# guomc9/CudaRayTracing

Measured on AMD Instinct MI355X. Metric: Mrays/sec, higher is better.
Workload: dtype f32

## Files before the change

cudaraytracing_amd/_capi.py:

```python
import ctypes as C
import os

import numpy as np

from . import build as _build

CRT_OK = 0
ERR_INVALID_ARG, ERR_NO_DEVICE, ERR_HIP = -1, -2, -3
TRAVERSAL_EXACT = 0
TRAVERSAL_REFERENCE = 1
TRAVERSAL_FAST = 2
FLAG_STATS = 1
FLAG_TILED_OUTPUT = 2
FLAG_FORCE_EXACT = 4
FLAG_TRACE_ALL = 8
FLAG_BOUNDED_RADIANCE = 16
FLAG_VARIANCE = 32
GATHER_AUTO, GATHER_RCCL, GATHER_COPY = 0, 1, 2
INTERSECT_RAW_DIRECTIONS, INTERSECT_FORCE_EXACT, INTERSECT_VISIBILITY = 0x100, 0x200, 0x400
TILE = 8


class CrtError(RuntimeError):
    def __init__(self, status, where, detail):
# ... 130 lines not shown
                ("width", C.c_uint32), ("height", C.c_uint32), ("bvh_thresh_n", C.c_uint32),
                ("light_sample_n", C.c_uint32), ("spp", C.c_uint32), ("p_rr", C.c_float)]


NODE_DTYPE = np.dtype([("lc", "<i4"), ("rc", "<i4"), ("n", "<u4"), ("it", "<i4"), ("aa", "<f4", 3), ("bb", "<f4", 3)])
TRI_DTYPE = np.dtype([("v1", "<f4", 3), ("v2", "<f4", 3), ("v3", "<f4", 3), ("normal", "<f4", 3), ("area", "<f4"),
                      ("area_of_obj", "<f4"), ("material", "<i4")])
MAT_DTYPE = np.dtype([("kd", "<f4", 3), ("ke", "<f4", 3), ("ns", "<f4"), ("mode", "<i4"), ("has_emit", "<i4")])
LIGHT_DTYPE = np.dtype([("first_tri", "<u4"), ("count", "<u4")])

ABI_VERSION = 5

EXPORTS = ["crt_strerror", "crt_last_error", "crt_abi_version", "crt_device_count", "crt_scene_create",
           "crt_scene_accel_info", "crt_scene_destroy", "crt_task_obj", "crt_shard_slots", "crt_render", "crt_render_device", "crt_render_range", "crt_render_range_device", "crt_last_launch_ms", "crt_radiance_storage", "crt_preview", "crt_preview_device", "crt_variance", "crt_variance_device", "crt_render_aov", "crt_render_aov_device", "crt_denoise_defaults", "crt_denoise_scratch_bytes", "crt_denoise", "crt_denoise_device", "crt_denoise_var_defaults", "crt_denoise_var", "crt_denoise_var_device", "crt_multi_create", "crt_multi_destroy",
           "crt_multi_render", "crt_multi_frame_device", "crt_intersect",
           "crt_device_math", "crt_device_philox", "crt_device_rcp_check", "crt_scene_export", "crt_host_scene_create", "crt_host_scene_destroy",
           "crt_host_scene_add_obj", "crt_host_scene_set_bvh", "crt_host_scene_set_bvh_device", "crt_host_scene_desc", "crt_host_scene_num_objects",
           "crt_host_scene_object", "crt_inverse_view", "crt_task_load", "crt_image_load", "crt_write_png", "crt_write_pfm"]

_lib = None


def lib_path():
    return _build.LIB


def lib():
    global _lib
    if _lib is not None:
        return _lib
    path = os.environ.get("CRT_LIB_PATH") or _build.build_lib()
# ... 33 lines not shown
    L.crt_denoise_var_defaults.argtypes = [C.POINTER(DenoiseParams)]
    L.crt_denoise_var.argtypes = [C.c_int, C.POINTER(DenoiseParams), C.POINTER(DenoiseVarInputs), C.c_void_p, C.c_void_p, C.c_void_p,
                                  C.POINTER(DenoiseInfo)]
    L.crt_denoise_var_device.argtypes = [C.c_int, C.POINTER(DenoiseParams), C.POINTER(DenoiseVarInputs), C.c_void_p, C.c_void_p, C.c_void_p,
                                         C.c_void_p, C.c_uint64, C.c_void_p, C.POINTER(DenoiseInfo)]
    L.crt_multi_create.argtypes = [C.POINTER(SceneDesc), C.POINTER(C.c_int), C.c_uint32, C.c_uint32, C.POINTER(C.c_void_p)]
    L.crt_multi_destroy.argtypes = [C.c_void_p]
    L.crt_multi_render.argtypes = [C.c_void_p, C.POINTER(Camera), C.POINTER(Params), C.c_void_p, C.c_void_p, C.POINTER(Stats),
                                   C.POINTER(MultiInfo)]
    L.crt_multi_frame_device.argtypes = [C.c_void_p, C.POINTER(C.c_void_p), C.POINTER(C.c_void_p), C.POINTER(C.c_int)]
    L.crt_intersect.argtypes = [C.c_void_p, C.c_uint32, C.c_void_p, C.c_void_p, C.c_uint32, C.c_void_p, C.c_void_p]
    L.crt_device_math.argtypes = [C.c_int, C.c_char_p, C.c_uint32, C.c_void_p, C.c_void_p, C.c_void_p]
    L.crt_device_philox.argtypes = [C.c_int, C.c_uint32, C.c_void_p, C.c_void_p, C.c_void_p]
    L.crt_device_rcp_check.argtypes = [C.c_int, C.POINTER(C.c_uint64), C.POINTER(C.c_uint64)]
    L.crt_scene_export.argtypes = [C.c_void_p, C.c_char_p, C.c_void_p, C.c_size_t, C.POINTER(C.c_size_t)]
    L.crt_host_scene_create.argtypes = [C.c_uint32, C.c_uint32, C.POINTER(C.c_void_p)]
    L.crt_host_scene_destroy.argtypes = [C.c_void_p]
    L.crt_host_scene_add_obj.argtypes = [C.c_void_p, C.c_char_p, C.c_char_p]
    L.crt_host_scene_set_bvh.argtypes = [C.c_void_p, C.c_uint32]
    L.crt_host_scene_set_bvh_device.argtypes = [C.c_void_p, C.c_uint32, C.c_int, C.POINTER(BvhBuildInfo)]
    L.crt_host_scene_desc.argtypes = [C.c_void_p, C.POINTER(SceneDesc)]
    L.crt_host_scene_num_objects.argtypes = [C.c_void_p, C.POINTER(C.c_uint32)]
    L.crt_host_scene_object.argtypes = [C.c_void_p, C.c_uint32, C.POINTER(C.c_float), C.POINTER(C.c_int32),
                                        C.POINTER(C.c_uint32)]
    L.crt_inverse_view.argtypes = [C.c_void_p, C.c_void_p, C.c_void_p, C.c_void_p]
    L.crt_task_load.argtypes = [C.c_char_p, C.POINTER(Task)]
    L.crt_task_obj.argtypes = [C.c_char_p, C.c_uint32, C.c_char_p, C.c_char_p, C.c_uint32]
    L.crt_image_load.argtypes = [C.c_char_p, C.POINTER(C.c_int32), C.POINTER(C.c_int32), C.POINTER(C.c_int32), C.c_void_p, C.c_uint64]
    L.crt_write_png.argtypes = [C.c_char_p, C.c_uint32, C.c_uint32, C.c_void_p]
    L.crt_write_pfm.argtypes = [C.c_char_p, C.c_uint32, C.c_uint32, C.c_uint32, C.c_void_p]
# ... 19 lines not shown
```

cudaraytracing_amd/api.py:

```python
import ctypes as C
import math
import os

import numpy as np

from . import _capi as capi


def get_inverse_view_matrix(eye_pos, lookat, up):
    e = np.asarray(eye_pos, dtype=np.float32)
    l = np.asarray(lookat, dtype=np.float32)
    u = np.asarray(up, dtype=np.float32)
    out = np.zeros(9, dtype=np.float32)
    capi.check(capi.lib().crt_inverse_view(capi.ptr(e), capi.ptr(l), capi.ptr(u), capi.ptr(out)), "crt_inverse_view")
    return out


def fov_to_radians(fov_y_deg):
    return np.float32(np.float32(np.float32(fov_y_deg) * np.float32(math.pi)) / np.float32(180))


class Task:

    def __init__(self, config_path, base_dir=None):
# ... 60 lines not shown
        buf = (C.c_char * (n * dtype.itemsize)).from_address(C.addressof(p.contents))
        return np.frombuffer(buf, dtype=dtype).copy()

    def nodes(self):
        d = self.desc()
        return self._arr(d.nodes, d.n_nodes, capi.NODE_DTYPE)

    def triangles(self):
        d = self.desc()
        return self._arr(d.tris, d.n_tris, capi.TRI_DTYPE)

    def light_triangles(self):
        d = self.desc()
        return self._arr(d.light_tris, d.n_light_tris, capi.TRI_DTYPE)

    def materials(self):
        d = self.desc()
        return self._arr(d.materials, d.n_materials, capi.MAT_DTYPE)

    def lights(self):
        d = self.desc()
        return self._arr(d.lights, d.n_lights, capi.LIGHT_DTYPE)

    @property
    def root(self):
        return int(self.desc().root)

    def objects(self):
        n = C.c_uint32()
        capi.check(capi.lib().crt_host_scene_num_objects(self._h, C.byref(n)), "crt_host_scene_num_objects")
# ... 44 lines not shown
        self.denoise_info = None
        self.variance_buffer = None

    def _handle(self, what):
        if not self._h:
            raise RuntimeError("%s: no single-device scene handle (freed, or a MultiRender)" % what)
        return self._h

    def accel_info(self):
        self._handle("accel_info")
        a = capi.AccelInfo()
        capi.check(capi.lib().crt_scene_accel_info(self._h, C.byref(a)), "crt_scene_accel_info")
        return a.as_dict()

    EXPORT_ARRAYS = {"nodes": np.float32, "nodes3": np.float32, "nodes4": np.float32, "nodes4i": np.float32, "leaf_geo": np.float32,
                     "leaf_geo_i": np.float32, "rec_map": np.int32, "tri_geo": np.float32, "leaf_count": np.int32, "tri_nm": np.float32}

    def export_trees(self):
        h = self._handle("export_trees")
        L = capi.lib()
        out = {}
        for name, dt in self.EXPORT_ARRAYS.items():
            n = C.c_size_t()
            capi.check(L.crt_scene_export(h, name.encode(), None, 0, C.byref(n)), "crt_scene_export")
            a = np.zeros(n.value // np.dtype(dt).itemsize, dtype=dt)
            if n.value:
                capi.check(L.crt_scene_export(h, name.encode(), capi.ptr(a), a.nbytes, C.byref(n)), "crt_scene_export")
            out[name] = a.reshape(-1, 4) if dt is np.float32 else a
        s = capi.TreeScalars()
        n = C.c_size_t()
        capi.check(L.crt_scene_export(h, b"scalars", C.byref(s), C.sizeof(s), C.byref(n)), "crt_scene_export")
# ... 446 lines not shown
```

cudaraytracing_amd/csrc/crt_device.h:

```cpp
#ifndef CRT_DEVICE_H
#define CRT_DEVICE_H

#include <hip/hip_runtime.h>
#include <stdint.h>

#include "crt_detmath.h"

namespace crtdev {

#define CRT_EPSILON 0.00001f
#define CRT_BOUNCE_STACK_SIZE 64
#define CRT_TILE 8

#define NODE4I_F4 6
#define TNM_MAT(w_) ((w_) & 0x3fffffffu)
#define TNM_EMITTER(w_) (((w_) >> 30) & 1u)
#define TNM_SPECULAR(w_) ((w_) >> 31)

struct DevScene {
    const float4* nodes;
    const float4* tri_geo;
    const int32_t* tri_mat;
    const float4* mats;
    const float4* ltri;
    const uint4* lights;
    const int32_t* leaf_count;
    int32_t root_fast;
    int32_t root_exact;
    int32_t n_lights;
    const float4* nodes3;
    const float4* leaf_geo;
    int32_t root3_fast, root3_exact;
// ... 92 lines not shown
```

cudaraytracing_amd/csrc/crt_mega3.hip:

```cpp
#include "crt_internal.h"

#include <cstdio>
#include <cstdlib>
#include <cstring>
#include <vector>

namespace crtk {

struct NewRay {
    F3 o, d;
    float tl;
    uint32_t kind, flags;
};

__device__ __forceinline__ float fmin3(float a, float b, float c) { return __builtin_fminf(__builtin_fminf(a, b), c); }
__device__ __forceinline__ float fmax3(float a, float b, float c) { return __builtin_fmaxf(__builtin_fmaxf(a, b), c); }
__device__ __forceinline__ v2f v2(float a, float b) { v2f r; r.x = a; r.y = b; return r; }
__device__ __forceinline__ v2f v2s(float a) { v2f r; r.x = a; r.y = a; return r; }

__device__ __forceinline__ int smax(const int a, const int b)
{
    int r;
    asm("s_max_i32 %0, %1, %2" : "=s"(r) : "s"(a), "s"(b) : "scc");
    return r;
// ... 128 lines not shown
            if (v - j >= 0) {
                F3 ind = mul3(L, f3(fm[j].x, fm[j].y, fm[j].z));
                ind = scale3(ind, cs[j]);
                ind = scale3(ind, inv_pdf_sphere);
                ind = div3(ind, P.p_rr);
                L = add3(ind, f3(a[j].x, a[j].y, a[j].z));
            }
        }
    }
    return L;
}

__device__ __forceinline__ bool shadow_blocked_bit(const bool tl_inf, const int tri) { return tri >= 0 || tl_inf; }
#define ST_TL_INF (1u << 12)

template <int MODE, bool RING = false>
__device__ __forceinline__ uint32_t logic_A(const LParams& P, const Tables<false>& tb, const uint32_t g, const float4 qa, const float4 qb, NewRay& nr,
                                            PathCounters& cnt, const bool trace_all)
{
    const DevScene& sc = P.sc;
    const Pool& pl = P.pool;
    constexpr bool TRI_CC = MODE != 1;
    const float4 la = gld(&pl.la[g]);
    const uint4 idv = load_path_id<RING, !TRI_CC>(P, g);
    const float4 cc = gld(&pl.cc[g]);
    const uint32_t st = __float_as_uint(la.w);
    const uint32_t stage = (st >> 8) & 15u;
    const uint32_t vtri_old = TRI_CC ? ((st & 0xfffu) == ((uint32_t)ST_HIT << 8) ? 0u : __float_as_uint(cc.w)) : idv.w;
    const float4 vn = gld(&sc.tri_nm[vtri_old]);
    const float res_t = qa.w;
    const int res_tri = __float_as_int(qb.w);
    const float4 gq_hit = gld(&sc.tri_nm[res_tri >= 0 ? res_tri : 0]);
    const uint32_t mat_old = min(TNM_MAT(__float_as_uint(vn.w)), P.n_mats - 1u);
    const uint32_t mat_cur = stage == ST_HIT ? TNM_MAT(__float_as_uint(gq_hit.w)) : mat_old;
    uint32_t tnm_cur = stage == ST_HIT ? __float_as_uint(gq_hit.w) : __float_as_uint(vn.w);
    float4 m0_cur = mat_row(tb, mat_cur, 0);
    const uint32_t n_nee = (uint32_t)(sc.n_lights * P.lsn);
    const uint32_t q_next = stage == ST_SHADOW ? (st >> 16) + 1 : 0u;
    uint4 lg_next = make_uint4(0u, 1u, 0u, 0u);
    if (n_nee > 0) {
        if (sc.n_lights == 1) {
            const crt_u4v_ l0_ = *(const __attribute__((address_space(4))) crt_u4v_*)tb.lights;
            lg_next = make_uint4(l0_.x, l0_.y, l0_.z, l0_.w);
        } else lg_next = gld(&tb.lights[fast_div(q_next < n_nee ? q_next : 0u, P.lsn_div.m, P.lsn_div.sh)]);
    }
    Lane s;
    s.depth = st & 255u; s.q = st >> 16; s.stage = stage;
    s.Ld = f3(la.x, la.y, la.z);
    s.nrm = f3(vn.x, vn.y, vn.z); s.mat = TNM_MAT(__float_as_uint(vn.w));
    s.pixel_index = idv.x; s.k = idv.y; s.item = idv.z;
    s.ro = f3(qa.x, qa.y, qa.z); s.tl = 0.0f;
    s.rd = f3(qb.x, qb.y, qb.z);
    s.pos = s.ro; s.vtri = vtri_old; s.c = f3(0.0f, 0.0f, 0.0f); s.kind = RAY_NONE;
    bool do_enter = false;
    if (stage == ST_SHADOW) {
        const bool blocked = TRI_CC ? shadow_blocked_bit((st & ST_TL_INF) != 0u, res_tri) : shadow_blocked<MODE>(cc.w, res_t, res_tri);
        if (!blocked) s.Ld = add3(s.Ld, f3(cc.x, cc.y, cc.z));
        s.q++;
    } else if (stage == ST_HIT) {
// ... 62 lines not shown
        if (TNM_SPECULAR(tnm_cur)) gst_rec(&pl.rec_b[(size_t)s.depth * pl.n + g], make_float4(s.rd.x, s.rd.y, s.rd.z, 0.0f));
        if (!TRI_CC) store_path_tri(P, g, s.vtri);
        if (TNM_EMITTER(tnm_cur)) {
            gst(&pl.la[g], make_float4(TRI_CC ? __uint_as_float(s.vtri) : 0.0f, 0.0f, 0.0f, __uint_as_float(s.depth | ((uint32_t)ST_FIN << 8) | (1u << 16))));
            return PH3_LC;
        }
        s.Ld = f3(0.0f, 0.0f, 0.0f);
        s.q = 0;
        if (n_nee == 0) {
            gst(&pl.la[g], make_float4(0.0f, 0.0f, 0.0f, __uint_as_float(s.depth | ((uint32_t)ST_NEED << 8))));
            if (TRI_CC) gst(&pl.cc[g].w, __uint_as_float(s.vtri));
            nr.o = s.pos;
            return PH3_LB;
        }
    }
    constexpr int LA_LOOP_MIN = 16;
    const float4 m0 = m0_cur;
    bool skip;
    for (bool first = true;; first = false) {
        if (first) setup_shadow_lg(P, s, f3(m0.x, m0.y, m0.z), lg_next);
        else setup_shadow(P, tb, s, f3(m0.x, m0.y, m0.z));
        skip = MODE != 1 && !trace_all && (s.c.x == 0.0f && s.c.y == 0.0f && s.c.z == 0.0f);
        if (!skip) break;
        cnt.untraced++;
        if (__popcll(__builtin_amdgcn_ballot_w64(true)) < LA_LOOP_MIN) break;
        cnt.rays++; cnt.shadow++;
        s.q++;
        if (s.q == n_nee) {
            gst(&pl.la[g], make_float4(s.Ld.x, s.Ld.y, s.Ld.z, __uint_as_float(s.depth | ((uint32_t)ST_NEED << 8))));
            if (TRI_CC) gst(&pl.cc[g].w, __uint_as_float(s.vtri));
            nr.o = s.pos;
            return PH3_LB;
        }
    }
    gst(&pl.la[g], make_float4(s.Ld.x, s.Ld.y, s.Ld.z, __uint_as_float(s.depth | ((uint32_t)ST_SHADOW << 8) | (s.q << 16) | ((TRI_CC && s.tl == pinf()) ? ST_TL_INF : 0u))));
    gst(&pl.cc[g], make_float4(s.c.x, s.c.y, s.c.z, TRI_CC ? __uint_as_float(s.vtri) : s.tl));
    nr.o = s.ro; nr.d = s.rd; nr.tl = s.tl; nr.kind = RAY_SHADOW;
    nr.flags = RF_SHADOW | (s.q + 1 == n_nee ? RF_LAST : 0u) | (skip ? RF_SKIP : 0u);
    return PH3_NONE;
}

template <int MODE, bool RING = false>
__device__ __forceinline__ uint32_t logic_B(const LParams& P, const uint32_t g, const float4 qa, const float4 qb, NewRay& nr)
{
    const Pool& pl = P.pool;
    constexpr bool TRI_CC = MODE != 1;
    const float4 la = gld(&pl.la[g]);
    const uint4 idv = load_path_id<RING, !TRI_CC>(P, g);
// ... 949 lines not shown
        } else {
            leaf_arm(std::true_type{});
        }
        }
      }
        if (act == PH3_NONE && !(commit_ring && (__builtin_amdgcn_readfirstlane((int)S.waitq) & 0xff) != 0)) break;
        STAMP_OTHER()
        if (act == PH3_LA) {
            POP3(PH3_LA)
            bool new_exact = false;
            if (on) {
                LOGIC_PARAMS()
                NewRay nr;
                float4 ra_, rb_;
                ray_result(S, id, ra_, rb_);
                nph = logic_A<MODE, RING>(Pl, tl, g, ra_, rb_, nr, cnt, ALL);
                if (nph == PH3_LB) { S.A[id].x = nr.o.x; S.A[id].y = nr.o.y; S.A[id].z = nr.o.z; }
                if (nph == PH3_NONE) nph = start_ray<MODE, false, LDS3, IMPL>(Pl.sc, S, id, nr, cnt, M3.force_exact != 0, new_exact);
            }
            n_exact += (int)__popcll(__ballot(new_exact));
            PUSH3()
            STAMP(0)
        } else if (act == PH3_LB) {
            POP3(PH3_LB)
            bool new_exact = false;
            if (on) {
                LOGIC_PARAMS()
                NewRay nr;
                float4 ra_, rb_;
                ray_result(S, id, ra_, rb_);
                nph = logic_B<MODE, RING>(Pl, g, ra_, rb_, nr);
// ... 94 lines not shown
            atomicAdd(&cs[C_TESTS], (unsigned long long)c);
            atomicAdd(&cs[C_HITS], (unsigned long long)d);
            atomicMax(&cs[C_MAXSP], (unsigned long long)ms);
            for (int p = 0; p < 5; p++) {
                atomicAdd(&cs[C_DIAG + 2 * p], (unsigned long long)dg_b[p]);
                atomicAdd(&cs[C_DIAG + 2 * p + 1], (unsigned long long)dg_l[p]);
            }
        }
        for (int k = 0; k < 6; k++) {
            const uint32_t v = wave_sum(dg_sp[k]);
            if (lane == 0) atomicAdd(&cs[C_DIAG + 10 + k], (unsigned long long)v);
        }
        for (int k = 0; k < 2; k++) {
            const uint32_t v = wave_sum(dg_ov[k]);
            if (lane == 0) atomicAdd(&cs[C_DIAG + 16 + k], (unsigned long long)v);
        }
    }
}

template <bool RING>
__global__ __launch_bounds__(64) void k_order_items(const LParams P, uint32_t* list, unsigned int* cnt)
{
    const uint32_t spans = (P.order_window + 1023u) / 1024u;
    const uint32_t sh = blockIdx.x / spans, sp = blockIdx.x - sh * spans;
    const uint32_t slo = sh * P.items_per_shard;
    if (slo >= P.n_items) return;
    const uint32_t hi = min(slo + P.items_per_shard, P.n_items);
    const uint32_t lo = hi - min(P.order_window, hi - slo);
    const uint32_t b = lo + sp * 1024u;
    if (b >= hi) return;
// ... 132 lines not shown
```

cudaraytracing_amd/csrc/crt_path.h:

```cpp
#ifndef CRT_PATH_H
#define CRT_PATH_H
#include "../../include/crt.h"
#include "crt_accel.h"
#include "crt_device.h"
#include "crt_trace.h"

#include <hip/hip_runtime.h>

#include <cfloat>
#include <cstddef>
#include <cstdint>
#include <type_traits>

namespace crtk {
using namespace crtdev;

enum { C_RAYS = 0, C_SHADOW, C_PROBE, C_INNER, C_LEAF, C_TESTS, C_HITS, C_PATHS, C_ALIVE, C_MAXSP, C_SUMSP, C_CYC_LOGIC, C_CYC_LEAF, C_CYC_INNER, C_CYC_OTHER,
       C_DIAG , C_UNTRACED = C_DIAG + 20, C_COUNT };
#define CNT_SHARDS 256
#define CNT_STRIDE 40
#define ITEM_SHARDS 64
#define ITEM_STRIDE 32

enum { ST_DEAD = 0, ST_NEW = 1, ST_HIT = 2, ST_PROBE = 3, ST_SHADOW = 4, ST_FIN = 5, ST_NEED = 6, ST_WAIT = 7, ST_COUNT_ };
// ... 134 lines not shown
        const int src = __ffsll((long long)found) - 1;
        const uint32_t sh = (uint32_t)__builtin_amdgcn_readlane((int)look, src);
        const int leader = __ffsll((long long)mask) - 1;
        unsigned int base = 0;
        if (lane == leader) base = __hip_atomic_fetch_add((CRT_GAS unsigned int*)(item_next + sh * ITEM_STRIDE), n, __ATOMIC_RELAXED, __HIP_MEMORY_SCOPE_AGENT);
        base = (unsigned int)__builtin_amdgcn_readlane((int)base, leader);
        const unsigned long long idx = (unsigned long long)base + rank;
        if (idx < per) { item = sh * per + (uint32_t)idx; break; }
    }
    return item;
}

struct PathCounters {
    uint32_t rays, shadow, probe, paths;
    uint32_t untraced;
};

struct Lane {
    F3 ro, rd, pos, Ld, c, nrm;
    float tl;
    uint32_t kind, vtri, mat, depth, stage, q, item;
    uint32_t pixel_index, k;
};

template <bool RING = false>
__device__ __forceinline__ void decode_item(const LParams& P, uint32_t item, uint32_t& pixel_index, uint32_t& k, bool& valid,
                                            uint32_t& pi, uint32_t& pj)
{
    uint32_t s, slot;
    if (RING) {
// ... 287 lines not shown
```

cudaraytracing_amd/csrc/crt_render.hip:

```cpp
#include "crt_internal.h"

#include <algorithm>
#include <cfloat>
#include <chrono>
#include <cstdio>
#include <cstdlib>
#include <cstring>
#include <limits>
#include <string>
#include <type_traits>
#include <array>
#include <atomic>
#include <vector>

using namespace crtdev;
using namespace crtk;

struct crt_scene {
    int device = 0;
    DevBuf<float4> nodes, tri_geo, mats, ltri, nodes3, leaf_geo, tri_nm, nodes4, nodes4i, leaf_geo_i;
    DevBuf<int32_t> rec_map;
    bool impl_ok = false;
    int depth4 = 1;
    bool ref16_ok = false;
// ... 15 lines not shown
    DevBuf<float4> ring_L;
    std::vector<unsigned int> ring_state_host;
    uint64_t last_radiance_bytes = 0;
    uint32_t last_ring_samples = 0;
    DevBuf<unsigned int> order_cnt;
    DevBuf<unsigned int> slot_next[2];
    DevBuf<int2> spill[2];
    hipStream_t aux_stream = nullptr;
    hipEvent_t ev_fork = nullptr, ev_join = nullptr;
    hipEvent_t ev_k0 = nullptr, ev_k1 = nullptr;
    uint32_t last_launches = 0;
    int n_cus = 0;
    unsigned long long* h_counters = nullptr;
    DevScene dev{};
    int stack_cap = 0;
    uint32_t n_tris = 0;
    crt_accel_info accel{};
    struct { uint32_t samples = 0, spp = 0, width = 0, height = 0, rank = 0, world = 1, tiled = 0; } acc;
    DevBuf<float> accum_q;
    struct { uint32_t samples = 0, spp = 0, width = 0, height = 0, rank = 0, world = 1, tiled = 0; bool valid = false; } var;
    std::vector<hipEvent_t> ev;
    ~crt_scene()
    {
        for (hipEvent_t e : ev) (void)hipEventDestroy(e);
        if (ev_k0) (void)hipEventDestroy(ev_k0);
        if (ev_k1) (void)hipEventDestroy(ev_k1);
        if (ev_fork) (void)hipEventDestroy(ev_fork);
        if (ev_join) (void)hipEventDestroy(ev_join);
        if (aux_stream) (void)hipStreamDestroy(aux_stream);
        if (h_counters) (void)hipHostFree(h_counters);
    }
// ... 147 lines not shown
                    if (owned[(uint32_t)n.it + k]) return fail(CRT_ERR_INVALID_ARG, "crt_scene_create: two leaves share a triangle");
                    owned[(uint32_t)n.it + k] = 1;
                }
            } else { todo.push_back(n.lc); todo.push_back(n.rc); }
        }
        if (visited != d->n_nodes) return fail(CRT_ERR_INVALID_ARG, "crt_scene_create: nodes that the root does not reach");
    }
    if (d->n_materials >= (1u << 30)) return fail(CRT_ERR_INVALID_ARG, "crt_scene_create: more than 2^30 - 1 materials (the triangle rows keep two flag bits beside the index)");
    for (uint32_t i = 0; i < d->n_tris; i++)
        if (d->tris[i].material < 0 || (uint32_t)d->tris[i].material >= d->n_materials) return fail(CRT_ERR_INVALID_ARG, "crt_scene_create: triangle material index out of range");
    for (uint32_t i = 0; i < d->n_light_tris; i++)
        if (d->light_tris[i].material < 0 || (uint32_t)d->light_tris[i].material >= d->n_materials) return fail(CRT_ERR_INVALID_ARG, "crt_scene_create: light triangle material index out of range");
    for (uint32_t i = 0; i < d->n_lights; i++)
        if (d->lights[i].count == 0 || (uint64_t)d->lights[i].first_tri + d->lights[i].count > d->n_light_tris) return fail(CRT_ERR_INVALID_ARG, "crt_scene_create: light range outside the light triangle array");
    return CRT_OK;
}

struct Shard {
    uint32_t tiles_x, tiles_y, n_tiles, local_tiles, nslots;
};
struct RingPlan { uint32_t samples, spsh, shards; };
Shard make_shard(uint32_t w, uint32_t h, uint32_t world)
{
    Shard s;
    s.tiles_x = (w + CRT_TILE - 1) / CRT_TILE;
    s.tiles_y = (h + CRT_TILE - 1) / CRT_TILE;
    s.n_tiles = s.tiles_x * s.tiles_y;
    s.local_tiles = (s.n_tiles + world - 1) / world;
    s.nslots = s.local_tiles * 64u;
    return s;
// ... 661 lines not shown
            float e1[3] = {t.v2[0] - t.v1[0], t.v2[1] - t.v1[1], t.v2[2] - t.v1[2]};
            float e2[3] = {t.v3[0] - t.v1[0], t.v3[1] - t.v1[1], t.v3[2] - t.v1[2]};
            geo[i * 3ull + 0] = make_float4(t.v1[0], t.v1[1], t.v1[2], e1[0]);
            geo[i * 3ull + 1] = make_float4(e1[1], e1[2], e2[0], e2[1]);
            geo[i * 3ull + 2] = make_float4(e2[2], t.normal[0], t.normal[1], t.normal[2]);
            tri_mat[i] = t.material;
        }
        for (uint32_t i = 0; i < d->n_materials; i++) {
            const crt_material& m = d->materials[i];
            const float pi_f = (float)3.14159265358979323846;
            int32_t flags = (m.has_emit ? 1 : 0) | (m.mode == 1 ? 2 : 0);
            mats[i * 3ull + 0] = make_float4(m.kd[0] / pi_f, m.kd[1] / pi_f, m.kd[2] / pi_f, m.ns);
            mats[i * 3ull + 1] = make_float4(m.kd[0], m.kd[1], m.kd[2], as_float(flags));
            mats[i * 3ull + 2] = make_float4(m.ke[0], m.ke[1], m.ke[2], 0.0f);
        }
        for (uint32_t i = 0; i < d->n_light_tris; i++) {
            const crt_triangle& t = d->light_tris[i];
            const crt_material& m = d->materials[t.material];
            ltri[i * 4ull + 0] = make_float4(t.v1[0], t.v1[1], t.v1[2], t.v2[0]);
            ltri[i * 4ull + 1] = make_float4(t.v2[1], t.v2[2], t.v3[0], t.v3[1]);
            ltri[i * 4ull + 2] = make_float4(t.v3[2], t.normal[0], t.normal[1], t.normal[2]);
            ltri[i * 4ull + 3] = make_float4(m.ke[0], m.ke[1], m.ke[2], t.area_of_obj);
        }
        std::vector<float4> leaf_geo, nodes3(nodes.size());
        std::vector<int32_t> rec_of_it(d->n_tris, -1);
        uint32_t max_leaf = 0;
        for (uint32_t i = 0; i < d->n_nodes; i++) {
            const crt_bvh_node& nn = d->nodes[i];
            if (!(nn.lc < 0 && nn.rc < 0)) continue;
            max_leaf = std::max(max_leaf, nn.n);
            rec_of_it[nn.it] = (int32_t)(leaf_geo.size() / 5);
            for (uint32_t k = 0; k < nn.n; k += 2) {
                const uint32_t ia = (uint32_t)nn.it + k, ib = k + 1 < nn.n ? ia + 1 : ia;
                const float4 a0 = geo[ia * 3ull], a1 = geo[ia * 3ull + 1], a2 = geo[ia * 3ull + 2];
                const float4 b0 = geo[ib * 3ull], b1 = geo[ib * 3ull + 1], b2 = geo[ib * 3ull + 2];
                leaf_geo.push_back(make_float4(a0.x, b0.x, a0.y, b0.y));
                leaf_geo.push_back(make_float4(a0.z, b0.z, a0.w, b0.w));
                leaf_geo.push_back(make_float4(a1.x, b1.x, a1.y, b1.y));
// ... 301 lines not shown
        sc->ref16_ok = n_nodes4 <= 32768 && leaf_geo.size() / 5 <= 32768;
        sc->ref16_inner_ok = n_nodes4 <= 32768;
        sc->dec_ok = leaf_geo.size() / 5 <= (size_t)LEAF_REC_MAX + 1;
        sc->accel.layout_caps = (sc->ref16_ok ? 1u : 0u) | (sc->ref16_inner_ok ? 2u : 0u) | (sc->dec_ok ? 4u : 0u) | (sc->impl_ok ? 8u : 0u);
        std::vector<float4> tri_nm(d->n_tris);
        for (uint32_t i = 0; i < d->n_tris; i++) {
            const crt_material& m = d->materials[d->tris[i].material];
            const int32_t w = (int32_t)((uint32_t)d->tris[i].material | (m.has_emit ? 1u << 30 : 0u) | (m.mode == 1 ? 1u << 31 : 0u));
            tri_nm[i] = make_float4(d->tris[i].normal[0], d->tris[i].normal[1], d->tris[i].normal[2], as_float(w));
        }
        sc->nodes3.upload(nodes3); sc->leaf_geo.upload(leaf_geo); sc->tri_nm.upload(tri_nm);
        sc->dev.tri_nm = sc->tri_nm.p;
        sc->max_leaf = max_leaf;
        sc->dev.nodes3 = sc->nodes3.p; sc->dev.leaf_geo = sc->leaf_geo.p;
        sc->dev.root3_fast = ref3(root_fast); sc->dev.root3_exact = ref3(root_exact);
        std::vector<uint4> lights(d->n_lights);
        for (uint32_t i = 0; i < d->n_lights; i++) {
            FastDiv fd = make_fastdiv(d->lights[i].count);
            lights[i] = make_uint4(d->lights[i].first_tri, d->lights[i].count, fd.m, fd.sh);
        }
        sc->nodes.upload(nodes); sc->tri_geo.upload(geo); sc->tri_mat.upload(tri_mat); sc->mats.upload(mats);
        sc->ltri.upload(ltri); sc->lights.upload(lights); sc->leaf_count.upload(leaf_count);
        sc->counters.alloc((size_t)CNT_SHARDS * CNT_STRIDE);
        sc->item_next.alloc((size_t)1024 * ITEM_STRIDE);
        sc->slot_next[0].alloc((size_t)SLOT_SHARDS * SLOT_STRIDE);
        sc->slot_next[1].alloc((size_t)SLOT_SHARDS * SLOT_STRIDE);
        HIP_CHECK(hipStreamCreateWithFlags(&sc->aux_stream, hipStreamNonBlocking));
        HIP_CHECK(hipEventCreateWithFlags(&sc->ev_fork, hipEventDisableTiming));
        HIP_CHECK(hipEventCreateWithFlags(&sc->ev_join, hipEventDisableTiming));
        HIP_CHECK(hipEventCreate(&sc->ev_k0));
        HIP_CHECK(hipEventCreate(&sc->ev_k1));
        {
            hipDeviceProp_t prop;
            HIP_CHECK(hipGetDeviceProperties(&prop, device));
            sc->n_cus = prop.multiProcessorCount > 0 ? prop.multiProcessorCount : 256;
        }
        HIP_CHECK(hipHostMalloc((void**)&sc->h_counters, (size_t)CNT_SHARDS * CNT_STRIDE * sizeof(unsigned long long), hipHostMallocDefault));
        sc->dev.nodes = sc->nodes.p; sc->dev.tri_geo = sc->tri_geo.p; sc->dev.tri_mat = sc->tri_mat.p; sc->dev.mats = sc->mats.p;
        sc->dev.ltri = sc->ltri.p; sc->dev.lights = sc->lights.p; sc->dev.leaf_count = sc->leaf_count.p;
        sc->dev.root_fast = root_fast; sc->dev.root_exact = root_exact; sc->dev.n_lights = (int32_t)d->n_lights;
        sc->n_tris = d->n_tris;
        sc->n_mats = d->n_materials;
        sc->stack_cap = std::max(depth + 2, 3 * sc->depth4 + 2);
        *out = sc;
        return CRT_OK;
    } catch (const HipFail& f) {
        delete sc;
        return fail_hip(f);
    } catch (const std::bad_alloc&) {
        delete sc;
        return fail(CRT_ERR_OOM, "crt_scene_create: out of host memory");
    }
}

int crt_scene_accel_info(crt_scene* sc, crt_accel_info* out)
{
    if (!sc || !out) return fail(CRT_ERR_INVALID_ARG, "crt_scene_accel_info: null argument");
    *out = sc->accel;
    return CRT_OK;
}

int crt_scene_export(crt_scene* sc, const char* name, void* dst, size_t capacity, size_t* bytes)
{
    if (!bytes) return fail(CRT_ERR_INVALID_ARG, "crt_scene_export: null bytes");
    static const char* names[] = {"nodes", "nodes3", "nodes4", "nodes4i", "leaf_geo", "leaf_geo_i", "rec_map", "tri_geo", "leaf_count", "tri_nm", "scalars"};
    int id = -1;
    for (int i = 0; name && i < 11; i++)
        if (std::strcmp(name, names[i]) == 0) id = i;
    if (id < 0) return fail(CRT_ERR_INVALID_ARG, std::string("crt_scene_export: unknown array ") + (name ? name : "(null)"));
    if (!sc) return fail(CRT_ERR_INVALID_ARG, "crt_scene_export: null scene");
    if (id == 10) {
        crt_tree_scalars s;
        std::memset(&s, 0, sizeof(s));
        s.root_fast = sc->dev.root_fast; s.root_exact = sc->dev.root_exact; s.root3_fast = sc->dev.root3_fast; s.root3_exact = sc->dev.root3_exact;
        s.root4 = sc->dev.root4; s.root4i = sc->impl_ok ? sc->dev.root4i : 0;
        s.n_mixed4i = sc->impl_ok ? sc->dev.n_mixed4i : 0; s.empty4_off = sc->dev.empty4_off; s.empty4i_off = sc->impl_ok ? sc->dev.empty4i_off : 0;
        s.coord_max = sc->dev.coord_max; s.stack_cap = (uint32_t)sc->stack_cap; s.node4i_f4 = NODE4I_F4;
        *bytes = sizeof(s);
        if (!dst) return CRT_OK;
        if (capacity < sizeof(s)) return fail(CRT_ERR_INVALID_ARG, "crt_scene_export: capacity below the size");
        std::memcpy(dst, &s, sizeof(s));
        return CRT_OK;
    }
    const bool leaf_root = sc->dev.root_fast < 0, impl = sc->impl_ok;
    const void* src = nullptr;
    size_t n = 0;
    switch (id) {
    case 0: src = sc->nodes.p; n = leaf_root ? 0 : sc->nodes.n * sizeof(float4); break;
    case 1: src = sc->nodes3.p; n = leaf_root ? 0 : sc->nodes3.n * sizeof(float4); break;
    case 2: src = sc->nodes4.p; n = sc->nodes4.n * sizeof(float4); break;
    case 3: src = sc->nodes4i.p; n = impl ? sc->nodes4i.n * sizeof(float4) : 0; break;
    case 4: src = sc->leaf_geo.p; n = sc->leaf_geo.n * sizeof(float4); break;
    case 5: src = sc->leaf_geo_i.p; n = impl ? sc->leaf_geo_i.n * sizeof(float4) : 0; break;
    case 6: src = sc->rec_map.p; n = impl ? sc->rec_map.n * sizeof(int32_t) : 0; break;
    case 7: src = sc->tri_geo.p; n = sc->tri_geo.n * sizeof(float4); break;
    case 8: src = sc->leaf_count.p; n = sc->leaf_count.n * sizeof(int32_t); break;
    default: src = sc->tri_nm.p; n = sc->tri_nm.n * sizeof(float4); break;
    }
    *bytes = n;
    if (!dst || n == 0) return CRT_OK;
    if (capacity < n) return fail(CRT_ERR_INVALID_ARG, "crt_scene_export: capacity below the size");
    try {
        HIP_CHECK(hipSetDevice(sc->device));
        HIP_CHECK(hipMemcpy(dst, src, n, hipMemcpyDeviceToHost));
        return CRT_OK;
    } catch (const HipFail& f) {
        return fail_hip(f);
    }
}

int crt_scene_destroy(crt_scene* sc)
// ... 340 lines not shown
```

include/crt.h:

```cpp
#ifndef CRT_H
#define CRT_H

#include <stddef.h>
#include <stdint.h>

#ifdef __cplusplus
extern "C" {
#endif

#define CRT_ABI_VERSION 5

typedef enum {
    CRT_OK = 0,
    CRT_ERR_INVALID_ARG = -1,
    CRT_ERR_NO_DEVICE = -2,
    CRT_ERR_HIP = -3,
    CRT_ERR_UNSUPPORTED = -4,
    CRT_ERR_IO = -5,
    CRT_ERR_PARSE = -6,
    CRT_ERR_OOM = -7
} crt_status;

const char* crt_strerror(int status);
const char* crt_last_error(void);
// ... 187 lines not shown
#define CRT_INTERSECT_VISIBILITY 0x400u
int crt_intersect(crt_scene* scene, uint32_t n, const float* origins, const float* dirs, uint32_t traversal,
                  int32_t* out_tri, float* out_t);

int crt_device_math(int device, const char* fn, uint32_t n, const float* a, const float* b, float* out);
int crt_device_philox(int device, uint32_t n, const uint32_t* ctr4, const uint32_t* key2, uint32_t* out4);
int crt_device_rcp_check(int device, uint64_t* mismatches, uint64_t* outside);
typedef struct {
    int32_t root_fast, root_exact, root3_fast, root3_exact, root4, root4i;
    uint32_t n_mixed4i, empty4_off, empty4i_off;
    float coord_max;
    uint32_t stack_cap;
    uint32_t node4i_f4;
} crt_tree_scalars;
int crt_scene_export(crt_scene* scene, const char* name, void* dst, size_t capacity, size_t* bytes);

typedef struct crt_host_scene crt_host_scene;

int crt_host_scene_create(uint32_t width, uint32_t height, crt_host_scene** out);
int crt_host_scene_destroy(crt_host_scene* scene);
int crt_host_scene_add_obj(crt_host_scene* scene, const char* obj_path, const char* mtl_dir);
int crt_host_scene_set_bvh(crt_host_scene* scene, uint32_t thresh_n);
typedef struct {
    uint32_t n_triangles, n_nodes, levels;
    uint32_t host_ranges;
    uint32_t host_triangles;
    uint32_t host_sorts;
    uint64_t host_sort_elements;
    float device_ms;
    float total_ms;
// ... 32 lines not shown
```

Measured before the change: 13300.

## Skip shadow rays to lights provably below or behind the shading point

Builds per-light conservative records on the host (bounding box, plane-offset range, flags) and appends them to the lights table. Before next-event estimation, a cheap test checks whether a light lies entirely below the surface hemisphere or behind the light's own plane, and if so skips its shadow samples without tracing them. The goal is to avoid tracing shadow rays that would contribute zero. In exchange it adds extra loads of the records, more divergence in logic_A, and diagnostic counters; the test uses conservative epsilons to avoid wrongly culling lights.

```diff
diff --git a/cudaraytracing_amd/_capi.py b/cudaraytracing_amd/_capi.py
--- a/cudaraytracing_amd/_capi.py
+++ b/cudaraytracing_amd/_capi.py
@@ -168,7 +168,7 @@
 EXPORTS = ["crt_strerror", "crt_last_error", "crt_abi_version", "crt_device_count", "crt_scene_create",
            "crt_scene_accel_info", "crt_scene_destroy", "crt_task_obj", "crt_shard_slots", "crt_render", "crt_render_device", "crt_render_range", "crt_render_range_device", "crt_last_launch_ms", "crt_radiance_storage", "crt_preview", "crt_preview_device", "crt_variance", "crt_variance_device", "crt_render_aov", "crt_render_aov_device", "crt_denoise_defaults", "crt_denoise_scratch_bytes", "crt_denoise", "crt_denoise_device", "crt_denoise_var_defaults", "crt_denoise_var", "crt_denoise_var_device", "crt_multi_create", "crt_multi_destroy",
            "crt_multi_render", "crt_multi_frame_device", "crt_intersect",
-           "crt_device_math", "crt_device_philox", "crt_device_rcp_check", "crt_scene_export", "crt_host_scene_create", "crt_host_scene_destroy",
+           "crt_device_math", "crt_device_philox", "crt_device_rcp_check", "crt_scene_export", "crt_light_records", "crt_host_scene_create", "crt_host_scene_destroy",
            "crt_host_scene_add_obj", "crt_host_scene_set_bvh", "crt_host_scene_set_bvh_device", "crt_host_scene_desc", "crt_host_scene_num_objects",
            "crt_host_scene_object", "crt_inverse_view", "crt_task_load", "crt_image_load", "crt_write_png", "crt_write_pfm"]
 
@@ -232,6 +232,8 @@
     L.crt_device_philox.argtypes = [C.c_int, C.c_uint32, C.c_void_p, C.c_void_p, C.c_void_p]
     L.crt_device_rcp_check.argtypes = [C.c_int, C.POINTER(C.c_uint64), C.POINTER(C.c_uint64)]
     L.crt_scene_export.argtypes = [C.c_void_p, C.c_char_p, C.c_void_p, C.c_size_t, C.POINTER(C.c_size_t)]
+    if hasattr(L, "crt_light_records"):
+        L.crt_light_records.argtypes = [C.c_void_p, C.c_void_p, C.c_void_p]
     L.crt_host_scene_create.argtypes = [C.c_uint32, C.c_uint32, C.POINTER(C.c_void_p)]
     L.crt_host_scene_destroy.argtypes = [C.c_void_p]
     L.crt_host_scene_add_obj.argtypes = [C.c_void_p, C.c_char_p, C.c_char_p]
diff --git a/cudaraytracing_amd/api.py b/cudaraytracing_amd/api.py
--- a/cudaraytracing_amd/api.py
+++ b/cudaraytracing_amd/api.py
@@ -98,6 +98,13 @@
         d = self.desc()
         return self._arr(d.light_tris, d.n_light_tris, capi.TRI_DTYPE)
 
+    def light_records(self):
+        d = self.desc()
+        ltri = np.zeros((d.n_light_tris * 4, 4), dtype=np.float32)
+        rec = np.zeros((d.n_lights * 3, 4), dtype=np.float32)
+        capi.check(capi.lib().crt_light_records(C.byref(d), capi.ptr(ltri), capi.ptr(rec)), "crt_light_records")
+        return ltri, rec
+
     def materials(self):
         d = self.desc()
         return self._arr(d.materials, d.n_materials, capi.MAT_DTYPE)
@@ -172,7 +179,8 @@
         return a.as_dict()
 
     EXPORT_ARRAYS = {"nodes": np.float32, "nodes3": np.float32, "nodes4": np.float32, "nodes4i": np.float32, "leaf_geo": np.float32,
-                     "leaf_geo_i": np.float32, "rec_map": np.int32, "tri_geo": np.float32, "leaf_count": np.int32, "tri_nm": np.float32}
+                     "leaf_geo_i": np.float32, "rec_map": np.int32, "tri_geo": np.float32, "leaf_count": np.int32, "tri_nm": np.float32,
+                     "ltri": np.float32, "light_rec": np.float32}
 
     def export_trees(self):
         h = self._handle("export_trees")
diff --git a/cudaraytracing_amd/csrc/crt_device.h b/cudaraytracing_amd/csrc/crt_device.h
--- a/cudaraytracing_amd/csrc/crt_device.h
+++ b/cudaraytracing_amd/csrc/crt_device.h
@@ -16,6 +16,12 @@
 #define TNM_MAT(w_) ((w_) & 0x3fffffffu)
 #define TNM_EMITTER(w_) (((w_) >> 30) & 1u)
 #define TNM_SPECULAR(w_) ((w_) >> 31)
+#define LREC_F4 3
+#define LREC_PLANAR 1u
+#define LREC_BOUNDED 2u
+#define LREC_FACING 4u
+#define LREC_VALUE_MAX 0x1p40f
+#define LREC_NSUM_MAX 2.0f
 
 struct DevScene {
     const float4* nodes;
diff --git a/cudaraytracing_amd/csrc/crt_mega3.hip b/cudaraytracing_amd/csrc/crt_mega3.hip
--- a/cudaraytracing_amd/csrc/crt_mega3.hip
+++ b/cudaraytracing_amd/csrc/crt_mega3.hip
@@ -166,7 +166,23 @@
 __device__ __forceinline__ bool shadow_blocked_bit(const bool tl_inf, const int tri) { return tri >= 0 || tl_inf; }
 #define ST_TL_INF (1u << 12)
 
-template <int MODE, bool RING = false>
+#define LDEAD_REL 0x1p-18f
+#define LDEAD_ABS 0x1p-40f
+__device__ __forceinline__ bool light_dead(const float4 r0, const float4 r1, const float4 r2, const F3 p, const F3 n, const F3 f_r)
+{
+    const uint32_t fl = __float_as_uint(r0.w);
+    const float ns = absf(n.x) + (absf(n.y) + absf(n.z));
+    const float fs = absf(f_r.x) + (absf(f_r.y) + absf(f_r.z));
+    const float M = fmax3(fmax3(absf(r0.x), absf(r0.y), absf(r0.z)), fmax3(absf(r1.x), absf(r1.y), absf(r1.z)), fmax3(absf(p.x), absf(p.y), absf(p.z)));
+    const float e = LDEAD_REL * M + LDEAD_ABS;
+    const bool usable = ((fl & LREC_BOUNDED) != 0u) & (ns >= 0x1p-10f) & (ns <= 0x1p10f) & (fs <= LREC_VALUE_MAX);
+    const F3 far = f3((n.x > 0.0f ? r1.x : r0.x) - p.x, (n.y > 0.0f ? r1.y : r0.y) - p.y, (n.z > 0.0f ? r1.z : r0.z) - p.z);
+    const bool below = dot3(n, far) < -(ns * e);
+    const bool behind = ((fl & LREC_FACING) != 0u) & (dot3(f3(r2.x, r2.y, r2.z), p) - r1.w < -(LREC_NSUM_MAX * e));
+    return usable & (below | behind);
+}
+
+template <int MODE, bool RING = false, bool STATS = false>
 __device__ __forceinline__ uint32_t logic_A(const LParams& P, const Tables<false>& tb, const uint32_t g, const float4 qa, const float4 qb, NewRay& nr,
                                             PathCounters& cnt, const bool trace_all)
 {
@@ -190,11 +206,32 @@
     const uint32_t n_nee = (uint32_t)(sc.n_lights * P.lsn);
     const uint32_t q_next = stage == ST_SHADOW ? (st >> 16) + 1 : 0u;
     uint4 lg_next = make_uint4(0u, 1u, 0u, 0u);
+#ifdef CRT_NO_NEE_PREDICATE
+    constexpr bool NEE_PRED = false;
+#else
+    constexpr bool NEE_PRED = MODE != 1;
+#endif
+    const bool pred_on = NEE_PRED && !trace_all;
+    float4 lr0 = make_float4(0.0f, 0.0f, 0.0f, 0.0f), lr1 = lr0, lr2 = lr0;
+    uint32_t li_next = 0;
     if (n_nee > 0) {
         if (sc.n_lights == 1) {
             const crt_u4v_ l0_ = *(const __attribute__((address_space(4))) crt_u4v_*)tb.lights;
             lg_next = make_uint4(l0_.x, l0_.y, l0_.z, l0_.w);
-        } else lg_next = gld(&tb.lights[fast_div(q_next < n_nee ? q_next : 0u, P.lsn_div.m, P.lsn_div.sh)]);
+            if (pred_on) {
+                const __attribute__((address_space(4))) crt_f4v_* lr_ = (const __attribute__((address_space(4))) crt_f4v_*)tb.lights;
+                const crt_f4v_ a_ = lr_[1], b_ = lr_[2], c_ = lr_[3];
+                lr0 = make_float4(a_.x, a_.y, a_.z, a_.w); lr1 = make_float4(b_.x, b_.y, b_.z, b_.w); lr2 = make_float4(c_.x, c_.y, c_.z, c_.w);
+            }
+        } else {
+            const uint32_t q0_ = q_next < n_nee ? q_next : 0u;
+            li_next = fast_div(q0_, P.lsn_div.m, P.lsn_div.sh);
+            lg_next = gld(&tb.lights[li_next]);
+            if (pred_on && q0_ == li_next * (uint32_t)P.lsn) {
+                const float4* lr_ = (const float4*)(tb.lights + sc.n_lights) + (size_t)li_next * LREC_F4;
+                lr0 = gld(lr_); lr1 = gld(lr_ + 1);
+            }
+        }
     }
     Lane s;
     s.depth = st & 255u; s.q = st >> 16; s.stage = stage;
@@ -287,11 +324,55 @@
             return PH3_LB;
         }
     }
-    constexpr int LA_LOOP_MIN = 16;
+#ifndef CRT_LA_LOOP_MIN
+#define CRT_LA_LOOP_MIN 16
+#endif
+    constexpr int LA_LOOP_MIN = CRT_LA_LOOP_MIN;
     const float4 m0 = m0_cur;
+    const auto to_roulette = [&]() -> uint32_t {
+        gst(&pl.la[g], make_float4(s.Ld.x, s.Ld.y, s.Ld.z, __uint_as_float(s.depth | ((uint32_t)ST_NEED << 8))));
+        if (TRI_CC) gst(&pl.cc[g].w, __uint_as_float(s.vtri));
+        nr.o = s.pos;
+        return PH3_LB;
+    };
+    bool lg_cur = true;
+    if (pred_on) {
+        const F3 f_r = f3(m0.x, m0.y, m0.z);
+        const auto answer = [&](const uint32_t q_end) {
+            const uint32_t n = q_end - s.q;
+            cnt.rays += n; cnt.shadow += n; cnt.untraced += n;
+            if constexpr (STATS) {
+                for (uint32_t q = s.q; q < q_end; q++) {
+                    Lane t = s;
+                    t.q = q;
+                    setup_shadow(P, tb, t, f_r);
+                    cnt.pred_dead++;
+                    cnt.pred_wrong += (t.c.x == 0.0f && t.c.y == 0.0f && t.c.z == 0.0f) ? 0u : 1u;
+                }
+            }
+            s.q = q_end;
+        };
+        if (sc.n_lights == 1) {
+            if (do_enter && light_dead(lr0, lr1, lr2, s.pos, s.nrm, f_r)) {
+                answer(n_nee);
+                return to_roulette();
+            }
+        } else if (s.q == li_next * (uint32_t)P.lsn) {
+            const float4* lrec_ = (const float4*)(tb.lights + sc.n_lights);
+            if (__float_as_uint(lr0.w) & LREC_FACING) lr2 = gld(lrec_ + (size_t)li_next * LREC_F4 + 2);
+            for (uint32_t li = li_next; light_dead(lr0, lr1, lr2, s.pos, s.nrm, f_r);) {
+                answer((li + 1) * (uint32_t)P.lsn);
+                if (s.q == n_nee) return to_roulette();
+                lg_cur = false;
+                li++;
+                const float4* lr_ = lrec_ + (size_t)li * LREC_F4;
+                lr0 = gld(lr_); lr1 = gld(lr_ + 1); lr2 = gld(lr_ + 2);
+            }
+        }
+    }
     bool skip;
     for (bool first = true;; first = false) {
-        if (first) setup_shadow_lg(P, s, f3(m0.x, m0.y, m0.z), lg_next);
+        if (first && lg_cur) setup_shadow_lg(P, s, f3(m0.x, m0.y, m0.z), lg_next);
         else setup_shadow(P, tb, s, f3(m0.x, m0.y, m0.z));
         skip = MODE != 1 && !trace_all && (s.c.x == 0.0f && s.c.y == 0.0f && s.c.z == 0.0f);
         if (!skip) break;
@@ -299,12 +380,7 @@
         if (__popcll(__builtin_amdgcn_ballot_w64(true)) < LA_LOOP_MIN) break;
         cnt.rays++; cnt.shadow++;
         s.q++;
-        if (s.q == n_nee) {
-            gst(&pl.la[g], make_float4(s.Ld.x, s.Ld.y, s.Ld.z, __uint_as_float(s.depth | ((uint32_t)ST_NEED << 8))));
-            if (TRI_CC) gst(&pl.cc[g].w, __uint_as_float(s.vtri));
-            nr.o = s.pos;
-            return PH3_LB;
-        }
+        if (s.q == n_nee) return to_roulette();
     }
     gst(&pl.la[g], make_float4(s.Ld.x, s.Ld.y, s.Ld.z, __uint_as_float(s.depth | ((uint32_t)ST_SHADOW << 8) | (s.q << 16) | ((TRI_CC && s.tl == pinf()) ? ST_TL_INF : 0u))));
     gst(&pl.cc[g], make_float4(s.c.x, s.c.y, s.c.z, TRI_CC ? __uint_as_float(s.vtri) : s.tl));
@@ -1284,7 +1360,7 @@
                 NewRay nr;
                 float4 ra_, rb_;
                 ray_result(S, id, ra_, rb_);
-                nph = logic_A<MODE, RING>(Pl, tl, g, ra_, rb_, nr, cnt, ALL);
+                nph = logic_A<MODE, RING, STATS>(Pl, tl, g, ra_, rb_, nr, cnt, ALL);
                 if (nph == PH3_LB) { S.A[id].x = nr.o.x; S.A[id].y = nr.o.y; S.A[id].z = nr.o.z; }
                 if (nph == PH3_NONE) nph = start_ray<MODE, false, LDS3, IMPL>(Pl.sc, S, id, nr, cnt, M3.force_exact != 0, new_exact);
             }
@@ -1409,6 +1485,10 @@
         for (int k = 0; k < 2; k++) {
             const uint32_t v = wave_sum(dg_ov[k]);
             if (lane == 0) atomicAdd(&cs[C_DIAG + 16 + k], (unsigned long long)v);
+        }
+        {
+            const uint32_t pd = wave_sum(cnt.pred_dead), pw = wave_sum(cnt.pred_wrong);
+            if (lane == 0) { atomicAdd(&cs[C_DIAG + 18], (unsigned long long)pd); atomicAdd(&cs[C_DIAG + 19], (unsigned long long)pw); }
         }
     }
 }
diff --git a/cudaraytracing_amd/csrc/crt_path.h b/cudaraytracing_amd/csrc/crt_path.h
--- a/cudaraytracing_amd/csrc/crt_path.h
+++ b/cudaraytracing_amd/csrc/crt_path.h
@@ -172,6 +172,7 @@
 struct PathCounters {
     uint32_t rays, shadow, probe, paths;
     uint32_t untraced;
+    uint32_t pred_dead, pred_wrong;
 };
 
 struct Lane {
diff --git a/cudaraytracing_amd/csrc/crt_render.hip b/cudaraytracing_amd/csrc/crt_render.hip
--- a/cudaraytracing_amd/csrc/crt_render.hip
+++ b/cudaraytracing_amd/csrc/crt_render.hip
@@ -2,6 +2,7 @@
 
 #include <algorithm>
 #include <cfloat>
+#include <cmath>
 #include <chrono>
 #include <cstdio>
 #include <cstdlib>
@@ -53,7 +54,7 @@
     unsigned long long* h_counters = nullptr;
     DevScene dev{};
     int stack_cap = 0;
-    uint32_t n_tris = 0;
+    uint32_t n_tris = 0, n_light_tris = 0;
     crt_accel_info accel{};
     struct { uint32_t samples = 0, spp = 0, width = 0, height = 0, rank = 0, world = 1, tiled = 0; } acc;
     DevBuf<float> accum_q;
@@ -231,6 +232,56 @@
     for (uint32_t i = 0; i < d->n_lights; i++)
         if (d->lights[i].count == 0 || (uint64_t)d->lights[i].first_tri + d->lights[i].count > d->n_light_tris) return fail(CRT_ERR_INVALID_ARG, "crt_scene_create: light range outside the light triangle array");
     return CRT_OK;
+}
+
+void fill_light_tris(const crt_scene_desc& d, std::vector<float4>& ltri)
+{
+    ltri.resize(d.n_light_tris * 4ull);
+    for (uint32_t i = 0; i < d.n_light_tris; i++) {
+        const crt_triangle& t = d.light_tris[i];
+        const crt_material& m = d.materials[t.material];
+        ltri[i * 4ull + 0] = make_float4(t.v1[0], t.v1[1], t.v1[2], t.v2[0]);
+        ltri[i * 4ull + 1] = make_float4(t.v2[1], t.v2[2], t.v3[0], t.v3[1]);
+        ltri[i * 4ull + 2] = make_float4(t.v3[2], t.normal[0], t.normal[1], t.normal[2]);
+        ltri[i * 4ull + 3] = make_float4(m.ke[0], m.ke[1], m.ke[2], t.area_of_obj);
+    }
+}
+
+std::vector<float4> make_light_records(const crt_scene_desc& d, const std::vector<float4>& ltri)
+{
+    std::vector<float4> rec(d.n_lights * (size_t)LREC_F4);
+    for (uint32_t li = 0; li < d.n_lights; li++) {
+        const uint32_t first = d.lights[li].first_tri, count = d.lights[li].count;
+        const float* f0 = &ltri[first * 4ull].x;
+        const float n[3] = {f0[9], f0[10], f0[11]};
+        float lo[3] = {f0[0], f0[1], f0[2]}, hi[3] = {f0[0], f0[1], f0[2]};
+        double dmin = 0.0, dmax = 0.0;
+        bool planar = true, bounded = true, any = false;
+        for (uint32_t t = 0; t < count; t++) {
+            const float* f = &ltri[(first + t) * 4ull].x;
+            for (int k = 0; k < 16; k++) bounded = bounded && std::isfinite(f[k]);
+            for (int k = 12; k < 16; k++) bounded = bounded && std::fabs(f[k]) <= LREC_VALUE_MAX;
+            planar = planar && std::memcmp(f + 9, f0 + 9, 12) == 0;
+            for (int v = 0; v < 3; v++) {
+                const float* x = f + 3 * v;
+                for (int a = 0; a < 3; a++) { if (x[a] < lo[a]) lo[a] = x[a]; if (x[a] > hi[a]) hi[a] = x[a]; }
+                const double dt = (double)n[0] * x[0] + ((double)n[1] * x[1] + (double)n[2] * x[2]);
+                if (!any || dt < dmin) dmin = dt;
+                if (!any || dt > dmax) dmax = dt;
+                any = true;
+            }
+        }
+        float fmin_ = (float)dmin, fmax_ = (float)dmax;
+        if ((double)fmin_ > dmin) fmin_ = std::nextafterf(fmin_, -INFINITY);
+        if ((double)fmax_ < dmax) fmax_ = std::nextafterf(fmax_, INFINITY);
+        const float nsum = std::fabs(n[0]) + (std::fabs(n[1]) + std::fabs(n[2]));
+        const bool facing = planar && bounded && nsum >= 0x1p-10f && nsum <= LREC_NSUM_MAX && std::isfinite(fmin_) && std::isfinite(fmax_);
+        const int32_t flags = (int32_t)((planar ? LREC_PLANAR : 0u) | (bounded ? LREC_BOUNDED : 0u) | (facing ? LREC_FACING : 0u));
+        rec[li * (size_t)LREC_F4 + 0] = make_float4(lo[0], lo[1], lo[2], as_float(flags));
+        rec[li * (size_t)LREC_F4 + 1] = make_float4(hi[0], hi[1], hi[2], fmin_);
+        rec[li * (size_t)LREC_F4 + 2] = make_float4(n[0], n[1], n[2], fmax_);
+    }
+    return rec;
 }
 
 struct Shard {
@@ -922,14 +973,8 @@
             mats[i * 3ull + 1] = make_float4(m.kd[0], m.kd[1], m.kd[2], as_float(flags));
             mats[i * 3ull + 2] = make_float4(m.ke[0], m.ke[1], m.ke[2], 0.0f);
         }
-        for (uint32_t i = 0; i < d->n_light_tris; i++) {
-            const crt_triangle& t = d->light_tris[i];
-            const crt_material& m = d->materials[t.material];
-            ltri[i * 4ull + 0] = make_float4(t.v1[0], t.v1[1], t.v1[2], t.v2[0]);
-            ltri[i * 4ull + 1] = make_float4(t.v2[1], t.v2[2], t.v3[0], t.v3[1]);
-            ltri[i * 4ull + 2] = make_float4(t.v3[2], t.normal[0], t.normal[1], t.normal[2]);
-            ltri[i * 4ull + 3] = make_float4(m.ke[0], m.ke[1], m.ke[2], t.area_of_obj);
-        }
+        fill_light_tris(*d, ltri);
+        const std::vector<float4> light_rec = make_light_records(*d, ltri);
         std::vector<float4> leaf_geo, nodes3(nodes.size());
         std::vector<int32_t> rec_of_it(d->n_tris, -1);
         uint32_t max_leaf = 0;
@@ -1261,11 +1306,12 @@
         sc->max_leaf = max_leaf;
         sc->dev.nodes3 = sc->nodes3.p; sc->dev.leaf_geo = sc->leaf_geo.p;
         sc->dev.root3_fast = ref3(root_fast); sc->dev.root3_exact = ref3(root_exact);
-        std::vector<uint4> lights(d->n_lights);
+        std::vector<uint4> lights(d->n_lights * (size_t)(1 + LREC_F4));
         for (uint32_t i = 0; i < d->n_lights; i++) {
             FastDiv fd = make_fastdiv(d->lights[i].count);
             lights[i] = make_uint4(d->lights[i].first_tri, d->lights[i].count, fd.m, fd.sh);
         }
+        if (d->n_lights) std::memcpy(&lights[d->n_lights], light_rec.data(), light_rec.size() * sizeof(float4));
         sc->nodes.upload(nodes); sc->tri_geo.upload(geo); sc->tri_mat.upload(tri_mat); sc->mats.upload(mats);
         sc->ltri.upload(ltri); sc->lights.upload(lights); sc->leaf_count.upload(leaf_count);
         sc->counters.alloc((size_t)CNT_SHARDS * CNT_STRIDE);
@@ -1286,7 +1332,7 @@
         sc->dev.nodes = sc->nodes.p; sc->dev.tri_geo = sc->tri_geo.p; sc->dev.tri_mat = sc->tri_mat.p; sc->dev.mats = sc->mats.p;
         sc->dev.ltri = sc->ltri.p; sc->dev.lights = sc->lights.p; sc->dev.leaf_count = sc->leaf_count.p;
         sc->dev.root_fast = root_fast; sc->dev.root_exact = root_exact; sc->dev.n_lights = (int32_t)d->n_lights;
-        sc->n_tris = d->n_tris;
+        sc->n_tris = d->n_tris; sc->n_light_tris = d->n_light_tris;
         sc->n_mats = d->n_materials;
         sc->stack_cap = std::max(depth + 2, 3 * sc->depth4 + 2);
         *out = sc;
@@ -1300,6 +1346,22 @@
     }
 }
 
+int crt_light_records(const crt_scene_desc* d, float* ltri_out, float* rec_out)
+{
+    const int rc = validate_desc(d);
+    if (rc != CRT_OK) return rc;
+    try {
+        std::vector<float4> ltri;
+        fill_light_tris(*d, ltri);
+        const std::vector<float4> rec = make_light_records(*d, ltri);
+        if (ltri_out && !ltri.empty()) std::memcpy(ltri_out, ltri.data(), ltri.size() * sizeof(float4));
+        if (rec_out && !rec.empty()) std::memcpy(rec_out, rec.data(), rec.size() * sizeof(float4));
+        return CRT_OK;
+    } catch (const std::bad_alloc&) {
+        return fail(CRT_ERR_OOM, "crt_light_records: out of host memory");
+    }
+}
+
 int crt_scene_accel_info(crt_scene* sc, crt_accel_info* out)
 {
     if (!sc || !out) return fail(CRT_ERR_INVALID_ARG, "crt_scene_accel_info: null argument");
@@ -1310,9 +1372,9 @@
 int crt_scene_export(crt_scene* sc, const char* name, void* dst, size_t capacity, size_t* bytes)
 {
     if (!bytes) return fail(CRT_ERR_INVALID_ARG, "crt_scene_export: null bytes");
-    static const char* names[] = {"nodes", "nodes3", "nodes4", "nodes4i", "leaf_geo", "leaf_geo_i", "rec_map", "tri_geo", "leaf_count", "tri_nm", "scalars"};
+    static const char* names[] = {"nodes", "nodes3", "nodes4", "nodes4i", "leaf_geo", "leaf_geo_i", "rec_map", "tri_geo", "leaf_count", "tri_nm", "scalars", "ltri", "light_rec"};
     int id = -1;
-    for (int i = 0; name && i < 11; i++)
+    for (int i = 0; name && i < 13; i++)
         if (std::strcmp(name, names[i]) == 0) id = i;
     if (id < 0) return fail(CRT_ERR_INVALID_ARG, std::string("crt_scene_export: unknown array ") + (name ? name : "(null)"));
     if (!sc) return fail(CRT_ERR_INVALID_ARG, "crt_scene_export: null scene");
@@ -1342,6 +1404,8 @@
     case 6: src = sc->rec_map.p; n = impl ? sc->rec_map.n * sizeof(int32_t) : 0; break;
     case 7: src = sc->tri_geo.p; n = sc->tri_geo.n * sizeof(float4); break;
     case 8: src = sc->leaf_count.p; n = sc->leaf_count.n * sizeof(int32_t); break;
+    case 11: src = sc->ltri.p; n = sc->n_light_tris * 4ull * sizeof(float4); break;
+    case 12: src = sc->lights.p + sc->dev.n_lights; n = (size_t)sc->dev.n_lights * LREC_F4 * sizeof(float4); break;
     default: src = sc->tri_nm.p; n = sc->tri_nm.n * sizeof(float4); break;
     }
     *bytes = n;
diff --git a/include/crt.h b/include/crt.h
--- a/include/crt.h
+++ b/include/crt.h
@@ -225,6 +225,7 @@
     uint32_t node4i_f4;
 } crt_tree_scalars;
 int crt_scene_export(crt_scene* scene, const char* name, void* dst, size_t capacity, size_t* bytes);
+int crt_light_records(const crt_scene_desc* desc, float* ltri_out, float* rec_out);
 
 typedef struct crt_host_scene crt_host_scene;
 
```

New measurement: 13410 (median of 6 runs). No clear change (+0.9%).
